# juanaldayparejo/archnemesis-dist

Hardware: AMD Instinct MI355X
Metric: forward-models/sec (10k nu x 100 layers) (higher is better)
Workload: dtype f64; 1 GPU; synthetic correlated-k nadir thermal-emission forward model: 10000 wavenumbers x 100 layers x 8 gases, G=20, k-table 20Px15T (BASELINE configs[1], SURVEY C2); parallelism=replicas x1 (independent forward models)

## Files before the change

### archnemesis_dist_amd/csrc/ansfm_api.hip

```cpp
#include "ansfm_table_kernels.hip.h"
#include "ansfm_rt_params.h"
#include "ansfm_ctx.hip.h"

using namespace ansfm;

extern "C" {

int ansfm_abi_version(void) { return ANSFM_ABI_VERSION; }

int ansfm_create(int device, ansfm_ctx **out)
{
    if (!out) return ANSFM_ERR_INVALID;
    *out = nullptr;
    int ndev = 0;
    if (hipGetDeviceCount(&ndev) != hipSuccess || ndev <= 0 || device < 0 || device >= ndev)
        return ANSFM_ERR_HIP;
    ansfm_ctx *ctx = new ansfm_ctx();
    ctx->device = device;
    if (hipSetDevice(device) != hipSuccess) { delete ctx; return ANSFM_ERR_HIP; }
    if (hipStreamCreateWithFlags(&ctx->own_stream, hipStreamNonBlocking) != hipSuccess) {
        delete ctx;
        return ANSFM_ERR_HIP;
    }
    ctx->stream = ctx->own_stream;
// ... 419 lines not shown
{
    ansfm_ctx *ctx = const_cast<ansfm_ctx *>(cctx);
    CHECK_CTX(ctx);
    if (!applied || !valid_bytes_nonzero) FAIL(ANSFM_ERR_INVALID, "last_merge_order: null argument");
    *applied = ctx->last_merge_ordered ? 1 : 0;
    *valid_bytes_nonzero = 0;
    if (!ctx->last_merge_ordered || ctx->d_flag.bytes < kFlagInts * sizeof(int)) return ANSFM_OK;
    HIPCHK(hipSetDevice(ctx->device));
    unsigned long long v = 0;
    HIPCHK(hipMemcpyAsync(&v, ctx->d_flag.as<int>() + kFlagTileCounter + 8 + 4, sizeof v, hipMemcpyDeviceToHost, ctx->stream));
    HIPCHK(hipStreamSynchronize(ctx->stream));
    *valid_bytes_nonzero = (int64_t)v;
    return ANSFM_OK;
}

int ansfm_last_merge_suffix(const ansfm_ctx *cctx, int64_t *rows, int64_t *rows_of_list_merges)
{
    ansfm_ctx *ctx = const_cast<ansfm_ctx *>(cctx);
    CHECK_CTX(ctx);
    if (!rows || !rows_of_list_merges) FAIL(ANSFM_ERR_INVALID, "last_merge_suffix: null argument");
    *rows = *rows_of_list_merges = 0;
    if (ctx->d_flag.bytes < kFlagInts * sizeof(int)) return ANSFM_OK;
    HIPCHK(hipSetDevice(ctx->device));
    unsigned long long v[kMergeTotals] = {0, 0, 0, 0};
    HIPCHK(hipMemcpyAsync(v, ctx->d_flag.as<int>() + kFlagTileCounter + 8, sizeof v, hipMemcpyDeviceToHost, ctx->stream));
    HIPCHK(hipStreamSynchronize(ctx->stream));
    *rows = (int64_t)v[3];
    *rows_of_list_merges = (int64_t)(v[1] - v[0]) * ctx->last_merge_G;
    return ANSFM_OK;
}

static void launch_w_to_last(hipStream_t st, unsigned n_batch, const double *src, double *dst, int W, int Wpad, int X1, int X2,
                             int swap12, double padval, size_t src_stride = 0, size_t dst_stride = 0)
{
    const int X = X1 * X2;
    dim3 grid((unsigned)(Wpad / 32), (unsigned)((X + 31) / 32), n_batch);
    hipLaunchKernelGGL(k_transpose_w_last, grid, dim3(32, 8), 0, st, src, dst, W, Wpad, X1, X2, swap12, padval, src_stride,
                       dst_stride);
}

static int read_unsorted(ansfm_ctx *ctx, int *flag)
{
    *flag = 0;
    HIPCHK(hipMemcpyAsync(flag, ctx->d_flag.as<int>() + 1, sizeof(int), hipMemcpyDeviceToHost, ctx->stream));
    HIPCHK(hipStreamSynchronize(ctx->stream));
    if (*flag & 2) FAIL(ANSFM_ERR_HIP, "merge kernel: dynamic LDS does not start at address 0 (unexpected code object layout)");
    *flag &= 1;
    return ANSFM_OK;
}

}
// ... 1194 lines not shown
```

### archnemesis_dist_amd/csrc/ansfm_ctx.hip.h

```cpp
#pragma once
#include <hip/hip_runtime.h>
#include <stdio.h>
#include <stdlib.h>
#include <string.h>

#include <algorithm>
#include <cmath>
#include <initializer_list>
#include <memory>
#include <string>
#include <map>
#include <vector>

#pragma GCC visibility push(default)
#include "../../include/ansfm.h"
#pragma GCC visibility pop
#include "ansfm_merge_plan.h"

namespace ansfm {

struct DevBuf {
    void *p = nullptr;
    size_t bytes = 0;
    DevBuf() = default;
// ... 19 lines not shown
    double t_ref = 0, p_ref = 0, s_floor = 0, wn_calc_window = 0, wn_approx_window = 0;
    DevBuf lines;
    std::vector<double> dabs;
    int Nb = 0, nb = 0;
    int first = 0, last = 0, jmax = 0;
    double t_cont = 0, p_cont = 0, wmax = 0;
    DevBuf bins;
};

struct FusedRoute {
    DevBuf ws;
    size_t scratch_bytes = 0;
    int recorded = 0;
    hipEvent_t ev[3] = {nullptr, nullptr, nullptr};
    double ms[2] = {0.0, 0.0};
};

}

using ansfm::DevBuf;
using ansfm::FusedRoute;
using ansfm::LblrtIso;

constexpr int kFlagInts = 32, kFlagTileCounter = 16, kMergeTotals = 4;
static_assert(kFlagTileCounter + 8 + 2 * kMergeTotals <= kFlagInts, "the totals lie inside d_flag");

struct ansfm_ctx {
    int device = 0;
    hipStream_t own_stream = nullptr;
    hipStream_t stream = nullptr;
    std::string err;
    int num_cus = 256;

    int W = 0, Wpad = 0, G = 0, NP = 0, NT = 0, S = 0;
    int monotone = 0;
    int has_boxed = 1;
    std::vector<double> h_wave, h_press, h_temp;
    DevBuf dcont_gas;
    int dcont_gas_L = 0;
    unsigned grad_gas_mask = 0xFFFFFFFFu;
    std::map<const void *, size_t> merge_lds_allowed;
    ansfm::MergePlan last_merge;
    int merge_keys = 64;
    DevBuf merge_hint;
    int merge_hint_parity = 0;
    struct MergeHintKey {
        long source = -1;
// ... 191 lines not shown
```

### archnemesis_dist_amd/csrc/ansfm_merge64.hip.h

```cpp
#pragma once
#include <hip/hip_runtime.h>
#include <stdint.h>
#include "ansfm_merge_common.hip.h"

namespace ansfm {

constexpr unsigned kLdsDG = 0, kLdsGORD = kMaxG * 8, kLdsDGF = (2 * kMaxG + 2) * 8, kLdsA = kLdsDGF + kMaxG * 4;


constexpr unsigned kLdsWT = kLdsA;
static_assert(kLdsA == kMergeLdsTables, "the plan's LDS arithmetic");
typedef double dbl2 __attribute__((ext_vector_type(2)));
constexpr unsigned kRecRow = 64u * 16u, kRecBin = 2u * kRecRow;

struct MergeElem {
    double ai, bc, bn, w;
    int ci, np;
};

struct MergeOrient {
    unsigned rbase, cbase;
    unsigned rsh, csh;
    unsigned inc;
};
// ... 339 lines not shown
#pragma unroll
            for (int j = 0; j < NR; ++j) {
                if (j < merge_rowmajor_sure_cols(NR) || j < G) {
                    MergeElem e;
                    e.ai = a0; e.bc = c[j]; e.w = lds_ld(wa + (unsigned)j * 256u);
                    merge_walk_nodiv(e, ws, rec);
                }
            }
        }
        return;
    }
    double w1[NR], a1;
    merge_rowmajor_weights<NR>(w0, a0, i0, G, mo);
    for (int i = i0; i < G; i += 2) {
        merge_rowmajor_weights<NR>(w1, a1, i + 1 < G ? i + 1 : i, G, mo);
        merge_rowmajor_row<NR>(a0, c, w0, G, ws, rec);
        if (i + 1 < G) {
            merge_rowmajor_weights<NR>(w0, a0, i + 2 < G ? i + 2 : i, G, mo);
            merge_rowmajor_row<NR>(a1, c, w1, G, ws, rec);
        }
    }
}

__device__ __forceinline__ void sort_column(double *X, unsigned char *P, int G, int lane)
{
    for (int g = 0; g < G; ++g) P[g * kWave + lane] = (unsigned char)g;
    for (int i = 1; i < G; ++i) {
        const double key = X[i * kWave + lane];
        const unsigned char pk = P[i * kWave + lane];
        int j = i - 1;
        while (j >= 0 && X[j * kWave + lane] > key) {
            X[(j + 1) * kWave + lane] = X[j * kWave + lane];
            P[(j + 1) * kWave + lane] = P[j * kWave + lane];
            --j;
        }
        X[(j + 1) * kWave + lane] = key;
        P[(j + 1) * kWave + lane] = pk;
    }
}

}
```

### archnemesis_dist_amd/csrc/ansfm_merge_common.hip.h

```cpp
#pragma once
#include <hip/hip_runtime.h>
#include <stdint.h>
#include "ansfm_merge_plan.h"

namespace ansfm {

__device__ __forceinline__ double encode_lnk(double k)
{
    if (k > 0.0) return log(k);
    unsigned long long b = (unsigned long long)__double_as_longlong(k);
    unsigned long long box = 0x7FF8000000000000ULL | (b >> 13);
    return __longlong_as_double((long long)box);
}
__device__ __forceinline__ bool lnk_is_boxed(double x) { return x != x; }
__device__ __forceinline__ double lnk_unbox(double x)
{
    unsigned long long b = (unsigned long long)__double_as_longlong(x);
    return __longlong_as_double((long long)((b & 0x0007FFFFFFFFFFFFULL) << 13));
}

struct LayerInterp {
    int ipl, iph, itl, ith;
    double v, u, dudt;
};
// ... 39 lines not shown
        double klo1 = lnk_unbox(l1), klo2 = lnk_unbox(l2), khi1 = lnk_unbox(h1), khi2 = lnk_unbox(h2);
        kk = (1.0 - v) * (1.0 - u) * klo1 + v * (1.0 - u) * khi1 + v * u * khi2 + (1.0 - v) * u * klo2;
        dk = (-klo1 * (1.0 - v) - khi1 * v + khi2 * v + klo2 * (1.0 - v)) * dudt;
    }
}


struct OverlapParams {
    const double *lnK;
    const double *kin;
    const LayerInterp *li;
    const double *amount;
    const double *del_g;
    double *tau;
    double *scratch;
    int *err_flag;
    unsigned int *tile_counter;
    int W, Wpad, G, NT, S, L, n_models;
    int delg_f32;
    double g_ord[kMaxG + 2];
    const double *lnKg;
    const unsigned char *hint_in;
    unsigned char *hint_out;
};
__host__ __device__ constexpr int gfast_stride(int G) { return (G + 1) & ~1; }
typedef double lnk_pair __attribute__((ext_vector_type(2)));


constexpr int kLoadBatch = 10;

template <bool FROM_K, bool NONNEG = false, bool NOBOX = false>
__device__ __forceinline__ void load_gas(const OverlapParams &p, const LayerInterp &q, int m, int l,
                                         int s, int nu, double *DST, int lane, bool &unsorted)
{
    const int G = p.G;
    const double amt = p.amount[((size_t)m * p.S + s) * p.L + l];
    double prev = NONNEG ? 0.0 : -__builtin_inf();
    if constexpr (FROM_K) {
        const double *src = p.kin + (((size_t)s * p.L + l) * G) * p.Wpad + nu;
        for (int g0 = 0; g0 < G; g0 += kLoadBatch) {
            double r[kLoadBatch];
#pragma unroll
            for (int k = 0; k < kLoadBatch; ++k) {
                const int gi = (g0 + k < G) ? g0 + k : G - 1;
                r[k] = src[(size_t)gi * p.Wpad];
            }
// ... 322 lines not shown
```

### archnemesis_dist_amd/csrc/ansfm_merge_plan.h

```cpp
#pragma once
#include <stddef.h>
#include <stdlib.h>
#include <string.h>

#include <type_traits>

#if defined(__HIPCC__)
#define ANSFM_HD __host__ __device__
#else
#define ANSFM_HD
#endif

namespace ansfm {

constexpr int kWave = 64;
constexpr int kMaxG = 32;

constexpr int kOptTable = 1, kOptBfi = 2, kOptExit = 8, kOptOrient = 16;
constexpr int kMergeOpt = kOptTable | kOptBfi | kOptExit | kOptOrient;
constexpr int kOptLaneRows = 32;
constexpr int kOptRowMajor = 64;
constexpr int kFlagLaneRows = 1, kFlagRowMajor = 2;
constexpr int kFlagTableGfast = 4;
constexpr int kFlagSuffixOff = 8;
ANSFM_HD constexpr bool merge_opt_valid(int opt) { return opt == 0 || (opt & ~kOptTable) == (kOptBfi | kOptExit | kOptOrient); }
ANSFM_HD constexpr int merge_wave_rows(int G, int opt) { return 2 * G + ((opt & kOptOrient) != 0 ? 2 : 1); }
constexpr int kMaxBlockWaves = 8;
ANSFM_HD constexpr unsigned weight_table_bytes(int G) { return (unsigned)(G + 1) * 32u * 8u; }
constexpr int kLaneNV = 2;

constexpr size_t kCuLdsBytes = (size_t)160 * 1024;
constexpr size_t kLdsGranule = 128;
constexpr size_t kMergeLdsTables = (size_t)(2 * kMaxG + 2) * sizeof(double) + kMaxG * sizeof(float);

inline int merge_list_len(int G)
{
    static const int sizes[] = {8, 10, 16, 20, 32};
    for (int v : sizes) if (v >= G) return v;
    return 32;
}
constexpr int kMergeOrderMinList = 16;
constexpr int kSuffixMinList = 16;
template <class F>
auto by_list_len(int G, F &&f)
{
    switch (merge_list_len(G)) {
        case 8: return f(std::integral_constant<int, 8>{});
        case 10: return f(std::integral_constant<int, 10>{});
        case 16: return f(std::integral_constant<int, 16>{});
        case 20: return f(std::integral_constant<int, 20>{});
        default: return f(std::integral_constant<int, 32>{});
    }
}

inline long merge_grid(int num_cus, size_t block_bytes, int max_per_cu, long ntiles)
{
    int per_cu = (int)(kCuLdsBytes / block_bytes);
    if (per_cu < 1) per_cu = 1;
    if (per_cu > max_per_cu) per_cu = max_per_cu;
    long grid = (long)num_cus * per_cu;
    if (grid > ntiles) grid = ntiles;
    return grid < 1 ? 1 : grid;
}

struct MergeSwitches {
    enum Lanes { kLanesUnset, kLanesWavenumbers, kLanesPairs };
    bool walk_records = false;
    bool load_boxtests = false;
    bool legacy = false;
    int keys = 0;
    int waves_per_cu = 0;
    Lanes lanes = kLanesUnset;
    bool rowmajor_off = false;
    bool layout_wave = false;
    bool order_off = false;
    bool suffix_off = false;
};
inline MergeSwitches merge_switches_from_env()
{
    MergeSwitches sw;
    const auto is = [](const char *name, const char *value) { const char *ev = getenv(name); return ev && !strcmp(ev, value); };
    const auto starts = [](const char *name, char c) { const char *ev = getenv(name); return ev && ev[0] == c; };
    sw.walk_records = is("ANSFM_MERGE_WALK", "records");
    sw.load_boxtests = starts("ANSFM_LOAD_BOXTESTS", '1');
    sw.legacy = starts("ANSFM_MERGE_LEGACY", '1');
    if (const char *ev = getenv("ANSFM_MERGE_KEYS")) sw.keys = atoi(ev) == 32 ? 32 : 64;
    if (const char *ev = getenv("ANSFM_WAVES_PER_CU")) sw.waves_per_cu = atoi(ev);
    if (is("ANSFM_MERGE_LANES", "wavenumbers")) sw.lanes = MergeSwitches::kLanesWavenumbers;
    else if (is("ANSFM_MERGE_LANES", "pairs")) sw.lanes = MergeSwitches::kLanesPairs;
    sw.rowmajor_off = starts("ANSFM_MERGE_ROWMAJOR", '0');
    sw.layout_wave = is("ANSFM_TABLE_LAYOUT", "wave");
    sw.order_off = starts("ANSFM_MERGE_ORDER", '0');
    sw.suffix_off = starts("ANSFM_MERGE_SUFFIX", '0');
    return sw;
}

struct MergeCall {
    bool from_k = false;
    bool generic = false;
    bool monotone = false;
    bool has_boxed = true;
    bool delg_f32 = false;
    int merge_keys = 64;
    int G = 0, S = 0, W = 0, Wpad = 0, L = 0, n_models = 0, num_cus = 0;
    double w00 = 0.0, g_ord1 = 0.0;
    bool gfast_copy = false;
    int table_W = 0, table_Wpad = 0, table_G = 0, table_S = 0;
    size_t lds32 = 0;
};

struct MergePlan {
    bool sorted = false, nodiv = false, nobox = false, keys32 = false;
    int opt = 0;
    bool lane_rows = false, rowmajor = false, gfast = false;
    bool suffix = false;
    int lane_nv = 0, flags = 0;
    bool order = false;
    int nwaves = 1;
    size_t lds = 0;
    long grid = 1;
    size_t scratch_bytes_per_block = 0;
    int trims = 0, group_width = 0;
};

inline MergePlan merge_plan(const MergeCall &c, const MergeSwitches &sw)
{
    MergePlan m;
    m.sorted = !c.generic && (c.from_k || c.monotone);
    m.nodiv = m.sorted && c.G >= 2 && c.w00 < c.g_ord1 && !sw.walk_records;
    m.nobox = m.nodiv && !c.from_k && !c.has_boxed && !sw.load_boxtests;
    m.keys32 = m.nodiv && (sw.keys != 0 ? sw.keys : c.merge_keys) == 32;
    const bool trimmed = m.nodiv && !sw.legacy && !m.keys32;
    m.opt = !trimmed ? 0 : c.delg_f32 ? kMergeOpt : (kMergeOpt & ~kOptTable);
    const bool table = (m.opt & kOptTable) != 0;

    const int max_per_cu = sw.waves_per_cu >= 1 && sw.waves_per_cu < kMaxBlockWaves ? sw.waves_per_cu : kMaxBlockWaves;
    const size_t wave_bytes = (size_t)merge_wave_rows(c.G, m.opt) * kWave * sizeof(double);
    const long ntiles = (long)c.n_models * (c.Wpad / kWave) * c.L;
    if (table) {
        const size_t shared_bytes = kMergeLdsTables + weight_table_bytes(c.G);
        const int fit = (int)((kCuLdsBytes - shared_bytes) / wave_bytes);
        m.nwaves = fit < max_per_cu ? fit : max_per_cu;
        m.lds = shared_bytes + (size_t)m.nwaves * wave_bytes;
        const long per_cu = merge_grid(c.num_cus, m.lds, 1, ntiles), needed = (ntiles + m.nwaves - 1) / m.nwaves;
        m.grid = per_cu < needed ? per_cu : needed;
    } else {
        m.nwaves = 1;
        m.lds = m.keys32 ? c.lds32 : wave_bytes + kMergeLdsTables + (m.sorted ? 0 : (size_t)2 * c.G * kWave);
        m.grid = merge_grid(c.num_cus, (m.lds + kLdsGranule - 1) / kLdsGranule * kLdsGranule, max_per_cu, ntiles);
    }
    m.scratch_bytes_per_block = (size_t)m.nwaves * 6 * c.G * kWave * sizeof(double);

    m.lane_rows = m.opt != 0 && (long)c.n_models * c.L < (1L << 24) && sw.lanes != MergeSwitches::kLanesWavenumbers;
    m.lane_nv = m.opt == 0 ? 0 : sw.lanes == MergeSwitches::kLanesPairs ? kLaneNV : 1;
    m.rowmajor = table && !sw.rowmajor_off;
    m.gfast = m.lane_rows && !c.from_k && c.gfast_copy && c.W == c.table_W && c.Wpad == c.table_Wpad && c.G == c.table_G &&
              c.S == c.table_S && !sw.layout_wave;
    m.order = m.rowmajor && m.lane_rows && m.lane_nv == 1 && merge_list_len(c.G) >= kMergeOrderMinList && !sw.order_off;
    m.suffix = m.rowmajor && !sw.suffix_off && merge_list_len(c.G) >= kSuffixMinList;
    m.flags = (m.lane_rows ? kFlagLaneRows : 0) | (m.rowmajor ? kFlagRowMajor : 0) | (m.gfast ? kFlagTableGfast : 0) |
              (m.rowmajor && sw.suffix_off ? kFlagSuffixOff : 0);
    m.trims = m.opt | (m.lane_rows ? kOptLaneRows : 0) | (m.rowmajor ? kOptRowMajor : 0);
    m.group_width = m.lane_rows ? m.lane_nv : 0;
    return m;
}

}
```

### archnemesis_dist_amd/csrc/ansfm_overlap.hip

```cpp
#include "ansfm_overlap_kernels.hip.h"
#include "ansfm_merge32_launch.h"
#include "ansfm_ctx.hip.h"

namespace ansfm {

void merge_params(ansfm_ctx *ctx, OverlapParams &p, const double *kin, int W, int Wpad, int G, int S, int L, int n_models,
                  const LayerInterp *li, const double *amount, const double *del_g_dev, const double *del_g_host, double *tau)
{
    p.lnK = ctx->lnK.as<double>();
    p.kin = kin;
    p.li = li;
    p.amount = amount;
    p.del_g = del_g_dev;
    p.tau = tau;
    p.err_flag = ctx->d_flag.as<int>() + 1;
    p.tile_counter = reinterpret_cast<unsigned int *>(ctx->d_flag.as<int>() + kFlagTileCounter);
    p.W = W; p.Wpad = Wpad; p.G = G; p.NT = ctx->NT; p.S = S; p.L = L; p.n_models = n_models;
    p.delg_f32 = ctx->delg_f32;
    double acc = 0.0;
    float accf = 0.0f;
    p.g_ord[0] = 0.0;
    for (int g = 0; g < G; ++g) {
        if (ctx->delg_f32) { accf += (float)del_g_host[g]; p.g_ord[g + 1] = (double)accf; }
        else { acc += del_g_host[g]; p.g_ord[g + 1] = acc; }
    }
    p.g_ord[G] = 1.0;
    p.g_ord[G + 1] = __builtin_nan("");
}

int merge_launch_begin(ansfm_ctx *ctx, const OverlapParams &p, long grid, std::initializer_list<MergeWorkspace> workspaces)
{
    for (const MergeWorkspace &w : workspaces) HIPCHK(w.buf->reserve((size_t)grid * w.bytes_per_block));
    HIPCHK(hipMemsetAsync(p.tile_counter, 0, (8 + 2 * kMergeTotals) * sizeof(unsigned int), ctx->stream));
    return ANSFM_OK;
}

using MergeKernel = void (*)(OverlapParams, int, int);

template <int D, bool FK, bool W32>
static MergeKernel overlap_kernel_of(const MergePlan &m)
{
    constexpr int kTrimmed = W32 ? kMergeOpt : (kMergeOpt & ~kOptTable);
    if (m.opt == kTrimmed) return m.nobox ? k_ck_overlap<D, false, W32, true, true, true, kTrimmed> : k_ck_overlap<D, FK, W32, true, true, false, kTrimmed>;
    if (m.opt != 0) return nullptr;
    if (m.nodiv) return m.nobox ? k_ck_overlap<D, false, W32, true, true, true> : k_ck_overlap<D, FK, W32, true, true>;
    return m.sorted ? k_ck_overlap<D, FK, W32, true> : k_ck_overlap<D, FK, W32, false>;
}

template <bool FK>
static MergeKernel overlap_kernel_fk(const MergePlan &m, bool w32, int G)
// ... 6 lines not shown

static MergeKernel overlap_kernel(const MergePlan &m, bool from_k, bool w32, int G)
{
    return from_k ? overlap_kernel_fk<true>(m, w32, G) : overlap_kernel_fk<false>(m, w32, G);
}

int launch_overlap(ansfm_ctx *ctx, bool from_k, const double *kin, int W, int Wpad, int G, int S,
                   int L, int n_models, const LayerInterp *li, const double *amount,
                   const double *del_g_dev, const double *del_g_host, double *tau, bool generic)
{
    OverlapParams p;
    memset(&p, 0, sizeof p);
    merge_params(ctx, p, kin, W, Wpad, G, S, L, n_models, li, amount, del_g_dev, del_g_host, tau);
    const bool w32 = ctx->delg_f32 != 0;
    MergeCall c;
    c.from_k = from_k; c.generic = generic; c.monotone = ctx->monotone != 0; c.has_boxed = ctx->has_boxed != 0; c.delg_f32 = w32;
    c.merge_keys = ctx->merge_keys;
    c.G = G; c.S = S; c.W = W; c.Wpad = Wpad; c.L = L; c.n_models = n_models; c.num_cus = ctx->num_cus;
    c.w00 = w32 ? (double)((float)del_g_host[0] * (float)del_g_host[0]) : del_g_host[0] * del_g_host[0];
    c.g_ord1 = p.g_ord[1];
    c.gfast_copy = ctx->lnKg_bytes != 0 && !ctx->is_lbl;
    c.table_W = ctx->W; c.table_Wpad = ctx->Wpad; c.table_G = ctx->G; c.table_S = ctx->S;
    c.lds32 = overlap32_lds_bytes(G, w32);
    const MergePlan m = merge_plan(c, merge_switches_from_env());

    const int rc = merge_launch_begin(ctx, p, m.grid, {{&ctx->scratch, m.scratch_bytes_per_block}});
    if (rc) return rc;
    p.scratch = ctx->scratch.as<double>();
    if (m.gfast) p.lnKg = ctx->lnKg.as<double>();
    ctx->last_merge = m;
    ctx->last_merge_G = G;
    ctx->last_merge_ordered = false;
    ansfm_ctx::MergeHintKey key;
    bool valid = false;
    if (m.order) {
        key.source = from_k ? 0 : ctx->table_generation;
        key.W = W; key.Wpad = Wpad; key.R = n_models * L; key.S = S; key.G = G;
        HIPCHK(ctx->merge_hint.reserve((size_t)2 * Wpad));
        valid = key == ctx->merge_hint_key;
        if (!valid) HIPCHK(hipMemsetAsync(ctx->merge_hint.p, 0, (size_t)2 * Wpad, ctx->stream));
        p.hint_in = ctx->merge_hint.as<unsigned char>() + (size_t)ctx->merge_hint_parity * Wpad;
        p.hint_out = ctx->merge_hint.as<unsigned char>() + (size_t)(1 - ctx->merge_hint_parity) * Wpad;
    }
    if (m.keys32) {
        HIPCHK(launch_overlap32(p, from_k, (unsigned)m.grid, ctx->stream));
        return ANSFM_OK;
// ... 22 lines not shown
```

### archnemesis_dist_amd/csrc/ansfm_overlap_kernels.hip.h

```cpp
#pragma once
#include "ansfm_merge64.hip.h"

namespace ansfm {


template <bool FROM_K, bool NOBOX, int OPT>
__device__ __forceinline__ void load_cell(const OverlapParams &p, int lane_rows, bool gfast, const LaneRow &lr, const LayerInterp &q, int m,
                                          int l, int s, int nu, double *DST, int lane, bool &unsorted)
{
    if constexpr (OPT != 0) {
        if (lane_rows != 0) {
            if (!FROM_K && gfast) load_gas_rows<FROM_K, NOBOX, true>(p, lr, s, DST, lane, unsorted);
            else load_gas_rows<FROM_K, NOBOX, false>(p, lr, s, DST, lane, unsorted);
            return;
        }
    }
    load_gas<FROM_K, false, NOBOX>(p, q, m, l, s, nu, DST, lane, unsorted);
}

template <int NR, bool FROM_K, bool W32, bool SORTED = true, bool NODIV = false, bool NOBOX = false, int OPT = 0>
__global__ __launch_bounds__((OPT & kOptTable) != 0 ? kWave * kMaxBlockWaves : kWave) __attribute__((amdgpu_waves_per_eu(1, 2)))
void k_ck_overlap(OverlapParams p, int flags, int lane_nv)
{
    static_assert(OPT == 0 || (SORTED && NODIV), "the fast path");
    static_assert(merge_opt_valid(OPT), "OPT == 0 || (OPT & ~kOptTable) == (kOptBfi | kOptExit | kOptOrient)");
    constexpr bool kTable = (OPT & kOptTable) != 0, kOrient = (OPT & kOptOrient) != 0;
    static_assert(!kTable || W32, "the weight table holds float32 products only (launch_overlap)");
    constexpr bool kSuffix = kTable && NR >= kSuffixMinList;
    const int lane_rows = kTable ? (flags & kFlagLaneRows) : flags;
    const bool gfast = !FROM_K && OPT != 0 && (flags & kFlagTableGfast) != 0;
    const unsigned nvs = lane_nv == 1 ? 0u : kLaneNVShift;
    unsigned n_rowmajor = 0, n_merged = 0;
    unsigned n_suffix = 0;
    const bool ordered = kTable && p.hint_in != nullptr;
    unsigned n_hints = 0;
    extern __shared__ double smem[];
    const int lane = kTable ? (int)(threadIdx.x & 63u) : (int)threadIdx.x;
    const int wv = kTable ? __builtin_amdgcn_readfirstlane((int)(threadIdx.x >> 6)) : 0;
    const int nwv = kTable ? (int)(blockDim.x >> 6) : 1;
    const int G = p.G;
    double *DG = smem;
    double *GORD = DG + kMaxG;
    double *A = reinterpret_cast<double *>(reinterpret_cast<char *>(GORD + kMaxG + 2) + kMaxG * sizeof(float));
    if constexpr (kTable) {
        double *WT = A;
        for (int idx = (int)threadIdx.x; idx < (G + 1) * 32; idx += (int)blockDim.x) {
            const int row = idx & 31, col = idx >> 5;
            double w = 0.0;
            if (row < G && col < G) w = (double)((float)p.del_g[row] * (float)p.del_g[col]);
            WT[idx] = w;
        }
        A = WT + (G + 1) * 32 + (size_t)wv * merge_wave_rows(G, OPT) * kWave;
    }
    double *B = A + (kOrient ? G + 1 : G) * kWave;
    unsigned char *PA = reinterpret_cast<unsigned char *>(B + (G + 1) * kWave);
    unsigned char *PB = PA + G * kWave;
    if (wv == 0 && lane < G) {
        DG[lane] = p.del_g[lane];
        const_cast<float *>(delg_f32_table(DG))[lane] = (float)p.del_g[lane];
    }
    if (wv == 0 && lane < G + 2) GORD[lane] = p.g_ord[lane];
    const double HUGE_KEY = __longlong_as_double(0x7FE0000000000000LL);
    B[G * kWave + lane] = HUGE_KEY;
    if constexpr (kOrient) A[G * kWave + lane] = HUGE_KEY;
    __syncthreads();
    double wsum = 0.0;
    for (int g = 0; g < G; ++g) wsum += DG[g];
    const double wtot = wsum * wsum;

    double *rec = p.scratch + ((size_t)blockIdx.x * nwv + wv) * 6 * G * kWave;
    TileQueue tq;
    tq.init();
    for (;;) {
        int vt = 0, m = 0, l = 0;
        LaneRow lr{};
// ... 16 lines not shown
            if (!tq.next(p, lane, vt, m, l)) break;
        }
        const int nu = vt * kWave + lane;
        LayerInterp q;
        if constexpr (!FROM_K) q = p.li[(size_t)m * p.L + l];
        bool unsorted = false;
        unsigned pattern = 0;

        load_cell<FROM_K, NOBOX, OPT>(p, lane_rows, gfast, lr, q, m, l, 0, nu, A, lane, unsorted);
        double alast = A[(G - 1) * kWave + lane];
        if constexpr (!SORTED) sort_column(A, PA, G, lane);
        for (int s = 1; s < p.S; ++s) {
            load_cell<FROM_K, NOBOX, OPT>(p, lane_rows, gfast, lr, q, m, l, s, nu, B, lane, unsorted);
            if constexpr (SORTED)
                if (__builtin_amdgcn_ballot_w64(unsorted) != 0) break;
            const double blast = B[(G - 1) * kWave + lane];
            if constexpr (!SORTED) sort_column(B, PB, G, lane);
            if constexpr (SORTED) alast = A[(G - 1) * kWave + lane];
            bool takeB, keepA;
            if (s == 1) { takeB = (alast <= 0.0); keepA = !takeB && (blast <= 0.0); }
            else { keepA = (blast <= 0.0); takeB = !keepA && (alast <= 0.0); }
            const bool do_merge = !(takeB | keepA);
            bool walked = false;
            int walked_rows = 0;
            if (takeB) {
                for (int g = 0; g < G; ++g) A[g * kWave + lane] = B[g * kWave + lane];
                if constexpr (!SORTED) {
                    for (int g = 0; g < G; ++g) PA[g * kWave + lane] = PB[g * kWave + lane];
                    alast = blast;
                }
            }
            if (do_merge) {
                double R[NR];
                MergeOrient mo{};
                if constexpr (kOrient) {
                    bool swapped = blast > alast;
                    if (__builtin_amdgcn_ballot_w64(swapped) != 0) {
                        double prev = A[lane];
                        for (int g = 1; g < G; ++g) {
                            const double v = A[g * kWave + lane];
                            swapped &= (v >= prev);
                            prev = v;
                        }
                    }
                    mo = merge_orient(lds_addr(A + lane), lds_addr(B + lane), swapped);
                    merge_init<NR>(R, G, mo, HUGE_KEY);
// ... 13 lines not shown
                    walked = i0 == 0;
                    if (i0 != 0) walked_rows = G - i0;
                    pattern |= lane_passes && s <= 8 ? 0x100u >> s : 0u;
                }
                if (!kTable || i0 != 0) {
                merge_fetch<W32, SORTED, OPT>(R[0], lane, A, B, DG, e0, PA, PB, mo);
                ws = walk_begin(GORD, lane);
                const bool partial = kSuffix && i0 < G;
                const int nloop = partial ? G * i0 : G * G - (G - 1);
                constexpr int kPer = 2;
                for (int n = nloop / kPer; n > 0; --n) {
                    merge_step<NR, W32, false, SORTED, NODIV, NR, OPT>(R, e0, e1, ws, lane, A, B, DG, GORD, rec, PA, PB, mo);
                    merge_step<NR, W32, false, SORTED, NODIV, NR, OPT>(R, e1, e0, ws, lane, A, B, DG, GORD, rec, PA, PB, mo);
                }
                if (!partial || (nloop & 1) != 0)
                merge_step<NR, W32, false, SORTED, NODIV, NR, OPT>(R, e0, e1, ws, lane, A, B, DG, GORD, rec, PA, PB, mo);
                if (!partial) {
                if (((G ^ NR) & 1) != 0) { const MergeElem t = e0; e0 = e1; e1 = t; }
                merge_peel<NR - 1, NR, W32, SORTED, NODIV, OPT>(R, e0, e1, ws, G, lane, A, B, DG, GORD, rec, PA, PB, mo);
                }
                }
                if constexpr (kTable) {
                    if (i0 < G) {
                        if (i0 == 0) ws = walk_begin(GORD, lane);
                        merge_rowmajor<NR>(i0, G, mo, ws, rec);
                    }
                }
                if constexpr (NODIV) {
                    const int ig = walk_bins(ws, GORD);
                    for (int g0 = 0; g0 < G; g0 += kLoadBatch) {
                        double r[kLoadBatch];
#pragma unroll
                        for (int k = 0; k < kLoadBatch; ++k)
                            r[k] = gld<double>(rec, (unsigned)((g0 + k < G) ? g0 + k : G - 1) * (kWave * 8u) + (unsigned)lane * 8u);
#pragma unroll
                        for (int k = 0; k < kLoadBatch; ++k) {
                            const int b = g0 + k;
                            if (b < G) {
                                double outv = 0.0;
                                if (b < ig) outv = fast_div(r[k], GORD[b + 1] - GORD[b]);
                                else if (b == ig) outv = (b == G - 1) ? fast_div(ws.kacc, ws.gd - GORD[G - 1]) : ws.kacc;
                                A[b * kWave + lane] = outv;
                            }
                        }
                    }
                } else {
                double ck = 0.0, cs = 0.0;
                const int ig = walk_bins(ws, GORD);
                constexpr int kRB = 5;
                for (int b0 = 0; b0 < G; b0 += kRB) {
                    double rka[kRB], rs1[kRB], rgd[kRB];
                    unsigned rcd[kRB];
#pragma unroll
                    for (int k = 0; k < kRB; ++k) {
                        const int bi = (b0 + k < G) ? b0 + k : G - 1;
                        const unsigned ro = (unsigned)bi * kRecBin + (unsigned)lane * 16u;
                        const dbl2 v0 = gld<dbl2>(rec, ro), v1 = gld<dbl2>(rec, ro + kRecRow);
                        rka[k] = v0.x; rs1[k] = v0.y; rgd[k] = v1.x; rcd[k] = (unsigned)__double_as_longlong(v1.y);
                    }
#pragma unroll
                    for (int k = 0; k < kRB; ++k) {
                        const int b = b0 + k;
                        if (b < G) {
// ... 12 lines not shown
                                const double kb = (ck + ka) + frac * cw;
                                const double sb = (cs + s1) + frac * w;
                                outv = fast_div(kb, sb);
                                ck = (1.0 - frac) * cw;
                                cs = (1.0 - frac) * w;
                            } else if (b == ig) {
                                const double kb = ck + ws.kacc, sb = cs + ws.sum1;
                                outv = (b == G - 1) ? fast_div(kb, sb) : kb;
                            }
                            gst<double>(rec, (unsigned)b * kRecBin + (unsigned)lane * 16u, outv);
                        }
                    }
                }
                for (int g0 = 0; g0 < G; g0 += kLoadBatch) {
                    double r[kLoadBatch];
#pragma unroll
                    for (int k = 0; k < kLoadBatch; ++k)
                        r[k] = gld<double>(rec, (unsigned)((g0 + k < G) ? g0 + k : G - 1) * kRecBin + (unsigned)lane * 16u);
#pragma unroll
                    for (int k = 0; k < kLoadBatch; ++k)
                        if (g0 + k < G) A[(g0 + k) * kWave + lane] = r[k];
                }
                }
                if constexpr (!SORTED) {
                    for (int g = 0; g < G; ++g) PA[g * kWave + lane] = (unsigned char)g;
                    alast = A[(G - 1) * kWave + lane];
                }
            }
            if constexpr (kTable) {
                n_merged += __builtin_amdgcn_ballot_w64(do_merge) != 0 ? 1u : 0u;
                n_rowmajor += __builtin_amdgcn_ballot_w64(walked) != 0 ? 1u : 0u;
                const unsigned long long some = __builtin_amdgcn_ballot_w64(walked_rows != 0);
                if (some != 0) n_suffix += (unsigned)__builtin_amdgcn_readlane(walked_rows, __builtin_ctzll(some));
            }
        }
        if constexpr (OPT != 0) {
            if (lane_rows != 0) {
                if (unsorted) atomicOr(p.err_flag, 1);
                double *outr = p.tau + ((size_t)lr.row * G) * p.Wpad + lr.nu;
                for (int g = 0; g < G; ++g) outr[(size_t)g * p.Wpad] = A[g * kWave + lane];
                if constexpr (kTable) {
                    if (ordered && lr.row == (((unsigned)p.n_models * (unsigned)p.L) >> 1) && lr.nu < p.W)
                        p.hint_out[lr.nu] = (unsigned char)pattern;
                }
                continue;
            }
        }
        double *out = p.tau + (((size_t)m * p.L + l) * G) * p.Wpad + nu;
        if constexpr (SORTED) {
            if (unsorted) atomicOr(p.err_flag, 1);
            for (int g = 0; g < G; ++g) out[(size_t)g * p.Wpad] = A[g * kWave + lane];
        } else {
            for (int g = 0; g < G; ++g) out[(size_t)PA[g * kWave + lane] * p.Wpad] = A[g * kWave + lane];
        }
    }
    if constexpr (kTable) {
        unsigned long long *cnt = reinterpret_cast<unsigned long long *>(p.tile_counter + 8);
        if (lane == 0) {
            atomicAdd(cnt, (unsigned long long)n_rowmajor);
            atomicAdd(cnt + 1, (unsigned long long)n_merged);
            if (ordered) atomicAdd(cnt + 2, (unsigned long long)n_hints);
            if (n_suffix != 0) atomicAdd(cnt + 3, (unsigned long long)n_suffix);
        }
    }
}

}
```

### archnemesis_dist_amd/engine.py

```python
import contextlib
import ctypes as C
import os
import numpy as np

from . import _lib

_f8 = np.float64


def _np(a, dtype=_f8):
    return None if a is None else np.ascontiguousarray(a, dtype=dtype)


def _is_f32(a):
    return getattr(a, "dtype", None) == np.float32


def _ptr(a):
    if a is None:
        return None
    if isinstance(a, np.ndarray):
        return a.ctypes.data_as(C.c_void_p)
    return C.c_void_p(a.data_ptr())

# ... 219 lines not shown
        w = C.c_int()
        self._check(self._lib.ansfm_last_merge_group_width(self._ctx, C.byref(w)), "last_merge_group_width")
        return int(w.value)

    def ktable_gfast(self):
        p, b = C.c_int(), C.c_int64()
        self._check(self._lib.ansfm_ktable_gfast(self._ctx, C.byref(p), C.byref(b)), "ktable_gfast")
        return bool(p.value), int(b.value)

    def last_merge_table_layout(self):
        g = C.c_int()
        self._check(self._lib.ansfm_last_merge_table_layout(self._ctx, C.byref(g)), "last_merge_table_layout")
        return bool(g.value)

    def last_merge_rowmajor(self):
        m, t = C.c_int64(), C.c_int64()
        self._check(self._lib.ansfm_last_merge_rowmajor(self._ctx, C.byref(m), C.byref(t)), "last_merge_rowmajor")
        return int(m.value), int(t.value)

    def last_merge_suffix(self):
        r, t = C.c_int64(), C.c_int64()
        self._check(self._lib.ansfm_last_merge_suffix(self._ctx, C.byref(r), C.byref(t)), "last_merge_suffix")
        return int(r.value), int(t.value)

    def last_merge_order(self):
        a, n = C.c_int(), C.c_int64()
        self._check(self._lib.ansfm_last_merge_order(self._ctx, C.byref(a), C.byref(n)), "last_merge_order")
        return bool(a.value), int(n.value)

    def calc_k(self, press, temp, grad=False):
        press = _np(press); temp = _np(temp)
        W, G, NP, NT, S = self.dims
        L = press.shape[0]
        k = np.empty((W, G, L, S)); dk = np.empty((W, G, L, S)) if grad else None
        self._check(self._lib.ansfm_calc_k(self._ctx, L, _ptr(press), _ptr(temp), _ptr(k), _ptr(dk)), "calc_k")
        return (k, dk) if grad else k

    def k_overlap(self, del_g, k_w_g_l_gas, amount_layer):
        self.set_f32_semantics(getattr(self, "grid_f32", False), _is_f32(del_g))
        del_g = _np(del_g); k = _np(k_w_g_l_gas); am = _np(amount_layer)
        W, G, L, S = k.shape
        if am.shape != (S, L):
            raise ValueError("amount_layer must be (NGAS, NLAYER)")
        tau = np.empty((W, G, L))
        self._check(self._lib.ansfm_k_overlap(self._ctx, W, G, L, S, _ptr(del_g), _ptr(k), _ptr(am), _ptr(tau)),
                    "k_overlap")
# ... 1345 lines not shown
```

### include/ansfm.h

```cpp
#ifndef ANSFM_H
#define ANSFM_H

#include <stdint.h>

#ifdef __cplusplus
extern "C" {
#endif

#define ANSFM_ABI_VERSION 1

#define ANSFM_OK 0
#define ANSFM_ERR_INVALID 1
#define ANSFM_ERR_HIP 2
#define ANSFM_ERR_NOTABLE 3
#define ANSFM_ERR_UNSORTED 4
#define ANSFM_ERR_UNSUPPORTED 5

#define ANSFM_MAX_NG 32
#define ANSFM_MAX_CONT_GRAD_SLOTS 48

typedef struct ansfm_ctx ansfm_ctx;

int ansfm_abi_version(void);

int ansfm_create(int device, ansfm_ctx **ctx);
void ansfm_destroy(ansfm_ctx *ctx);
const char *ansfm_last_error(const ansfm_ctx *ctx);

int ansfm_set_stream(ansfm_ctx *ctx, void *hip_stream);
int ansfm_synchronize(ansfm_ctx *ctx);

int ansfm_set_f32_semantics(ansfm_ctx *ctx, int grid_f32, int delg_f32);

int ansfm_upload_ktable(ansfm_ctx *ctx, int W, int G, int NP, int NT, int S, const double *K,
                        const double *PRESS, const double *TEMP, const double *WAVE,
                        const double *DELG);
int ansfm_upload_ktable_dev(ansfm_ctx *ctx, int W, int G, int NP, int NT, int S,
                            const double *K_dev, const double *PRESS, const double *TEMP,
                            const double *WAVE, const double *DELG);
int ansfm_ktable_info(const ansfm_ctx *ctx, int64_t dims[5], int *monotone);
int ansfm_ktable_has_boxed(const ansfm_ctx *ctx, int *has_boxed);
int ansfm_last_merge_launch(const ansfm_ctx *ctx, int *waves_per_block, int *trims);
int ansfm_last_merge_rowmajor(const ansfm_ctx *ctx, int64_t *merges, int64_t *merges_total);
int ansfm_last_merge_suffix(const ansfm_ctx *ctx, int64_t *rows, int64_t *rows_of_list_merges);
int ansfm_last_merge_group_width(const ansfm_ctx *ctx, int *width);
int ansfm_ktable_gfast(const ansfm_ctx *ctx, int *present, int64_t *bytes);
int ansfm_last_merge_table_layout(const ansfm_ctx *ctx, int *gfast);
int ansfm_last_merge_order(const ansfm_ctx *ctx, int *applied, int64_t *valid_bytes_nonzero);

int ansfm_upload_lbltable(ansfm_ctx *ctx, int W, int NP, int NT, int S, const double *K,
                          const double *PRESS, const double *TEMP, int temp2d, const double *WAVE);
int ansfm_calc_klbl(ansfm_ctx *ctx, int L, const double *press, const double *temp, double *k_out,
                    double *dkdT_out);

int ansfm_ktable_file_header(const char *path, int64_t dims[4], int32_t ids[2], double hdr[3], double *wave,
                             float *g_ord, float *del_g, float *press, float *temp);
int ansfm_upload_ktable_files(ansfm_ctx *ctx, int S, const char *const *paths, double wavemin, double wavemax);
int ansfm_ktable_grids(const ansfm_ctx *ctx, double *WAVE, double *PRESS, double *TEMP, double *DELG);
int ansfm_lbltable_file_header(const char *path, int64_t dims[3], int32_t ids[2], double hdr[2], double *wave,
                               float *press, float *temp);
int ansfm_upload_lbltable_files(ansfm_ctx *ctx, int S, const char *const *paths, double wavemin, double wavemax);

int ansfm_kdist_bins(ansfm_ctx *ctx, int ncalc, const double *wavecalc, const double *kabs, int nbin,
                     const double *vbinmin, const double *vbinmax, const double *wcen, int nfilmax,
                     const int32_t *nfil, const double *dfil, const double *afil, int NG, const double *g_ord,
                     double *kout);

// ... 366 lines not shown
```

Before: 301.3 forward-models/s.

## Precompute static bin-crossing tables for random-overlap merge walk

On the host, it precomputes which (i,j) product cells cross each g-ordinate bin boundary, plus the split coefficients, for the float32 weight table. This is valid because the weights depend only on del_g. The kernel stores these tables and reciprocal bin widths in LDS and walks the merge with a uniform per-row bitmask, instead of doing data-dependent comparisons against the cumulative g-ordinates. Division by bin width is replaced with a refined reciprocal multiply. The change adds extra LDS per block, which may reduce waves per CU, and it only applies when G is at least 16 and the table is valid.

```diff
diff --git a/archnemesis_dist_amd/csrc/ansfm_api.hip b/archnemesis_dist_amd/csrc/ansfm_api.hip
--- a/archnemesis_dist_amd/csrc/ansfm_api.hip
+++ b/archnemesis_dist_amd/csrc/ansfm_api.hip
@@ -465,11 +465,27 @@
     *rows = *rows_of_list_merges = 0;
     if (ctx->d_flag.bytes < kFlagInts * sizeof(int)) return ANSFM_OK;
     HIPCHK(hipSetDevice(ctx->device));
-    unsigned long long v[kMergeTotals] = {0, 0, 0, 0};
+    unsigned long long v[4] = {0, 0, 0, 0};
     HIPCHK(hipMemcpyAsync(v, ctx->d_flag.as<int>() + kFlagTileCounter + 8, sizeof v, hipMemcpyDeviceToHost, ctx->stream));
     HIPCHK(hipStreamSynchronize(ctx->stream));
     *rows = (int64_t)v[3];
     *rows_of_list_merges = (int64_t)(v[1] - v[0]) * ctx->last_merge_G;
+    return ANSFM_OK;
+}
+
+int ansfm_last_merge_static(const ansfm_ctx *cctx, int64_t *merges, int *valid)
+{
+    ansfm_ctx *ctx = const_cast<ansfm_ctx *>(cctx);
+    CHECK_CTX(ctx);
+    if (!merges || !valid) FAIL(ANSFM_ERR_INVALID, "last_merge_static: null argument");
+    *merges = 0;
+    *valid = ctx->last_merge.static_tables ? 1 : 0;
+    if (ctx->d_flag.bytes < kFlagInts * sizeof(int)) return ANSFM_OK;
+    HIPCHK(hipSetDevice(ctx->device));
+    unsigned long long v = 0;
+    HIPCHK(hipMemcpyAsync(&v, ctx->d_flag.as<int>() + kFlagTileCounter + 8 + 8, sizeof v, hipMemcpyDeviceToHost, ctx->stream));
+    HIPCHK(hipStreamSynchronize(ctx->stream));
+    *merges = (int64_t)v;
     return ANSFM_OK;
 }
 
diff --git a/archnemesis_dist_amd/csrc/ansfm_ctx.hip.h b/archnemesis_dist_amd/csrc/ansfm_ctx.hip.h
--- a/archnemesis_dist_amd/csrc/ansfm_ctx.hip.h
+++ b/archnemesis_dist_amd/csrc/ansfm_ctx.hip.h
@@ -65,7 +65,7 @@
 using ansfm::FusedRoute;
 using ansfm::LblrtIso;
 
-constexpr int kFlagInts = 32, kFlagTileCounter = 16, kMergeTotals = 4;
+constexpr int kFlagInts = 40, kFlagTileCounter = 16, kMergeTotals = 5;
 static_assert(kFlagTileCounter + 8 + 2 * kMergeTotals <= kFlagInts, "the totals lie inside d_flag");
 
 struct ansfm_ctx {
diff --git a/archnemesis_dist_amd/csrc/ansfm_merge64.hip.h b/archnemesis_dist_amd/csrc/ansfm_merge64.hip.h
--- a/archnemesis_dist_amd/csrc/ansfm_merge64.hip.h
+++ b/archnemesis_dist_amd/csrc/ansfm_merge64.hip.h
@@ -385,6 +385,111 @@
     }
 }
 
+constexpr unsigned kStaticRD = 0, kStaticC = kMaxG * 16u, kStaticMask = 2u * kMaxG * 16u;
+static_assert(kStaticMask + kMaxG * 4u == kMergeStaticLds, "the plan's LDS arithmetic");
+__device__ __forceinline__ unsigned merge_static_base(int G) { return kLdsWT + weight_table_bytes(G); }
+typedef __attribute__((address_space(3))) dbl2 lds_dbl2;
+typedef __attribute__((address_space(3))) unsigned lds_uint;
+__device__ __forceinline__ dbl2 lds_ld2(unsigned a) { return *(const lds_dbl2 *)(size_t)a; }
+__device__ __forceinline__ double recip_div(double n, dbl2 rd)
+{
+    const double q = n * rd.x;
+    return fma(fma(-rd.y, q, n), rd.x, q);
+}
+__device__ __forceinline__ void merge_static_fill(const OverlapParams &p, int G, int lane)
+{
+    const unsigned sb = merge_static_base(G);
+    if (lane < G) {
+        const double d = p.g_ord[lane + 1] - p.g_ord[lane];
+        double r = __builtin_amdgcn_rcp(d);
+        r = fma(fma(-d, r, 1.0), r, r);
+        r = fma(fma(-d, r, 1.0), r, r);
+        *(lds_dbl2 *)(size_t)(sb + kStaticRD + (unsigned)lane * 16u) = dbl2{r, d};
+    }
+    if (lane < kMaxG) {
+        *(lds_dbl2 *)(size_t)(sb + kStaticC + (unsigned)lane * 16u) = dbl2{p.st.c1[lane], p.st.c2[lane]};
+        *(lds_uint *)(size_t)(sb + kStaticMask + (unsigned)lane * 4u) = p.st.rowmask[lane];
+    }
+}
+struct StaticWalk {
+    double kacc;
+    dbl2 cc;
+    unsigned caddr;
+    unsigned oaddr;
+};
+template <bool TEST>
+__device__ __forceinline__ void merge_static_elem(int j, double cv, double w, unsigned mask, StaticWalk &sw)
+{
+    if (TEST && ((mask >> j) & 1u) != 0) {
+        lds_st(sw.oaddr, fma(sw.cc.x, cv, sw.kacc));
+        sw.kacc = sw.cc.y * cv;
+        sw.oaddr += 512u;
+        sw.caddr += 16u;
+        sw.cc = lds_ld2(sw.caddr);
+    } else
+        sw.kacc = fma(cv, w, sw.kacc);
+}
+template <int NR>
+__device__ __forceinline__ void merge_static_row(double ai, const double (&c)[NR], const double (&w)[NR], unsigned wa, unsigned mask,
+                                                 int G, StaticWalk &sw)
+{
+    constexpr int kSure = merge_rowmajor_sure_cols(NR);
+    constexpr unsigned kInner = ((1u << kSure) - 1u) & ~1u;
+    const auto weight = [&](int j) { if constexpr (NR > 20) return lds_ld(wa + (unsigned)j * 256u); else return w[j]; };
+    merge_static_elem<true>(0, ai + c[0], weight(0), mask, sw);
+    if ((mask & kInner) == 0) {
+#pragma unroll
+        for (int j = 1; j < kSure; ++j) merge_static_elem<false>(j, ai + c[j], weight(j), mask, sw);
+    } else {
+#pragma unroll
+        for (int j = 1; j < kSure; ++j) merge_static_elem<true>(j, ai + c[j], weight(j), mask, sw);
+    }
+#pragma unroll
+    for (int j = kSure; j < NR; ++j)
+        if (j < G) merge_static_elem<true>(j, ai + c[j], weight(j), mask, sw);
+}
+__device__ __forceinline__ unsigned merge_static_mask(unsigned sb, int i)
+{
+    return *(const lds_uint *)(size_t)(sb + kStaticMask + ((unsigned)i << 2));
+}
+template <int NR>
+__device__ __forceinline__ double merge_rowmajor_static(int G, const MergeOrient &mo, unsigned a_lane)
+{
+    const unsigned sb = merge_static_base(G);
+    double c[NR], w0[NR], a0;
+#pragma unroll
+    for (int j = 0; j < NR; ++j) c[j] = lds_ld(mo.cbase + (unsigned)(j < G ? j : 0) * 512u);
+    StaticWalk sw;
+    sw.kacc = 0.0;
+    sw.caddr = sb + kStaticC;
+    sw.cc = lds_ld2(sw.caddr);
+    sw.oaddr = a_lane;
+    if constexpr (NR > 20) {
+        for (int i = 0; i < G; ++i) {
+            a0 = lds_ld(mo.rbase + ((unsigned)i << 9));
+            const unsigned m = (unsigned)__builtin_amdgcn_readfirstlane((int)merge_static_mask(sb, i));
+            merge_static_row<NR>(a0, c, c, kLdsWT + ((unsigned)i << 3), m, G, sw);
+        }
+        return sw.kacc;
+    }
+    double w1[NR], a1;
+    unsigned m0 = merge_static_mask(sb, 0), m1;
+    merge_rowmajor_weights<NR>(w0, a0, 0, G, mo);
+    for (int i = 0; i < G; i += 2) {
+        const int i1 = i + 1 < G ? i + 1 : i;
+        m1 = merge_static_mask(sb, i1);
+        merge_rowmajor_weights<NR>(w1, a1, i1, G, mo);
+        merge_static_row<NR>(a0, c, w0, 0u, (unsigned)__builtin_amdgcn_readfirstlane((int)m0), G, sw);
+        if (i + 1 < G) {
+            const int i2 = i + 2 < G ? i + 2 : i;
+            m0 = merge_static_mask(sb, i2);
+            merge_rowmajor_weights<NR>(w0, a0, i2, G, mo);
+            merge_static_row<NR>(a1, c, w1, 0u, (unsigned)__builtin_amdgcn_readfirstlane((int)m1), G, sw);
+        }
+    }
+    return sw.kacc;
+}
+
 __device__ __forceinline__ void sort_column(double *X, unsigned char *P, int G, int lane)
 {
     for (int g = 0; g < G; ++g) P[g * kWave + lane] = (unsigned char)g;
diff --git a/archnemesis_dist_amd/csrc/ansfm_merge_common.hip.h b/archnemesis_dist_amd/csrc/ansfm_merge_common.hip.h
--- a/archnemesis_dist_amd/csrc/ansfm_merge_common.hip.h
+++ b/archnemesis_dist_amd/csrc/ansfm_merge_common.hip.h
@@ -85,6 +85,7 @@
     const double *lnKg;
     const unsigned char *hint_in;
     unsigned char *hint_out;
+    MergeStatic st;
 };
 __host__ __device__ constexpr int gfast_stride(int G) { return (G + 1) & ~1; }
 typedef double lnk_pair __attribute__((ext_vector_type(2)));
diff --git a/archnemesis_dist_amd/csrc/ansfm_merge_plan.h b/archnemesis_dist_amd/csrc/ansfm_merge_plan.h
--- a/archnemesis_dist_amd/csrc/ansfm_merge_plan.h
+++ b/archnemesis_dist_amd/csrc/ansfm_merge_plan.h
@@ -1,4 +1,5 @@
 #pragma once
+#include <float.h>
 #include <stddef.h>
 #include <stdlib.h>
 #include <string.h>
@@ -23,6 +24,7 @@
 constexpr int kFlagLaneRows = 1, kFlagRowMajor = 2;
 constexpr int kFlagTableGfast = 4;
 constexpr int kFlagSuffixOff = 8;
+constexpr int kFlagStatic = 16, kFlagStaticOff = 32;
 ANSFM_HD constexpr bool merge_opt_valid(int opt) { return opt == 0 || (opt & ~kOptTable) == (kOptBfi | kOptExit | kOptOrient); }
 ANSFM_HD constexpr int merge_wave_rows(int G, int opt) { return 2 * G + ((opt & kOptOrient) != 0 ? 2 : 1); }
 constexpr int kMaxBlockWaves = 8;
@@ -41,6 +43,59 @@
 }
 constexpr int kMergeOrderMinList = 16;
 constexpr int kSuffixMinList = 16;
+constexpr int kStaticMinList = 16;
+constexpr size_t kMergeStaticLds = (size_t)kMaxG * 16 + (size_t)kMaxG * 16 + (size_t)kMaxG * 4;
+
+inline void merge_g_ord(const double *del_g, int G, bool delg_f32, double *g_ord)
+{
+    double acc = 0.0;
+    float accf = 0.0f;
+    g_ord[0] = 0.0;
+    for (int g = 0; g < G; ++g) {
+        if (delg_f32) { accf += (float)del_g[g]; g_ord[g + 1] = (double)accf; }
+        else { acc += del_g[g]; g_ord[g + 1] = acc; }
+    }
+    g_ord[G] = 1.0;
+    g_ord[G + 1] = __builtin_nan("");
+}
+
+struct MergeStatic {
+    unsigned rowmask[kMaxG];
+    double c1[kMaxG], c2[kMaxG];
+    double gd_end, last_width;
+    int nbins;
+    int valid;
+};
+inline void merge_static_build(const double *del_g, const double *g_ord, int G, MergeStatic &s)
+{
+    memset(&s, 0, sizeof s);
+    if (G < 2 || G > kMaxG) return;
+    const auto plain = [](float v) { const float m = v < 0.0f ? -v : v; return v == 0.0f || (m >= FLT_MIN && m <= FLT_MAX); };
+    bool ok = true;
+    double gd = 0.0;
+    int ig = 0;
+    for (int i = 0; i < G; ++i) {
+        for (int j = 0; j < G; ++j) {
+            const float fi = (float)del_g[i], fj = (float)del_g[j];
+            const float wf = fi * fj;
+            ok = ok && plain(fi) && plain(fj) && plain(wf);
+            const double w = (double)wf;
+            const double gdn = gd + w;
+            if (ig < G && gdn >= g_ord[ig + 1]) {
+                ok = ok && ig <= i;
+                s.rowmask[i] |= 1u << j;
+                s.c1[ig] = g_ord[ig + 1] - gd;
+                s.c2[ig] = gdn - g_ord[ig + 1];
+                ++ig;
+            }
+            gd = gdn;
+        }
+    }
+    s.nbins = ig;
+    s.gd_end = gd;
+    s.last_width = gd - g_ord[G - 1];
+    s.valid = ok ? 1 : 0;
+}
 template <class F>
 auto by_list_len(int G, F &&f)
 {
@@ -75,6 +130,7 @@
     bool layout_wave = false;
     bool order_off = false;
     bool suffix_off = false;
+    bool static_off = false;
 };
 inline MergeSwitches merge_switches_from_env()
 {
@@ -92,6 +148,7 @@
     sw.layout_wave = is("ANSFM_TABLE_LAYOUT", "wave");
     sw.order_off = starts("ANSFM_MERGE_ORDER", '0');
     sw.suffix_off = starts("ANSFM_MERGE_SUFFIX", '0');
+    sw.static_off = starts("ANSFM_MERGE_STATIC", '0');
     return sw;
 }
 
@@ -107,6 +164,7 @@
     bool gfast_copy = false;
     int table_W = 0, table_Wpad = 0, table_G = 0, table_S = 0;
     size_t lds32 = 0;
+    bool static_valid = false;
 };
 
 struct MergePlan {
@@ -114,6 +172,7 @@
     int opt = 0;
     bool lane_rows = false, rowmajor = false, gfast = false;
     bool suffix = false;
+    bool static_tables = false, static_walk = false;
     int lane_nv = 0, flags = 0;
     bool order = false;
     int nwaves = 1;
@@ -138,7 +197,8 @@
     const size_t wave_bytes = (size_t)merge_wave_rows(c.G, m.opt) * kWave * sizeof(double);
     const long ntiles = (long)c.n_models * (c.Wpad / kWave) * c.L;
     if (table) {
-        const size_t shared_bytes = kMergeLdsTables + weight_table_bytes(c.G);
+        m.static_tables = c.static_valid && merge_list_len(c.G) >= kStaticMinList;
+        const size_t shared_bytes = kMergeLdsTables + weight_table_bytes(c.G) + (m.static_tables ? kMergeStaticLds : 0);
         const int fit = (int)((kCuLdsBytes - shared_bytes) / wave_bytes);
         m.nwaves = fit < max_per_cu ? fit : max_per_cu;
         m.lds = shared_bytes + (size_t)m.nwaves * wave_bytes;
@@ -158,8 +218,10 @@
               c.S == c.table_S && !sw.layout_wave;
     m.order = m.rowmajor && m.lane_rows && m.lane_nv == 1 && merge_list_len(c.G) >= kMergeOrderMinList && !sw.order_off;
     m.suffix = m.rowmajor && !sw.suffix_off && merge_list_len(c.G) >= kSuffixMinList;
+    m.static_walk = m.static_tables && m.rowmajor && !sw.static_off;
     m.flags = (m.lane_rows ? kFlagLaneRows : 0) | (m.rowmajor ? kFlagRowMajor : 0) | (m.gfast ? kFlagTableGfast : 0) |
-              (m.rowmajor && sw.suffix_off ? kFlagSuffixOff : 0);
+              (m.rowmajor && sw.suffix_off ? kFlagSuffixOff : 0) | (m.static_tables ? kFlagStatic : 0) |
+              (m.static_tables && !m.static_walk ? kFlagStaticOff : 0);
     m.trims = m.opt | (m.lane_rows ? kOptLaneRows : 0) | (m.rowmajor ? kOptRowMajor : 0);
     m.group_width = m.lane_rows ? m.lane_nv : 0;
     return m;
diff --git a/archnemesis_dist_amd/csrc/ansfm_overlap.hip b/archnemesis_dist_amd/csrc/ansfm_overlap.hip
--- a/archnemesis_dist_amd/csrc/ansfm_overlap.hip
+++ b/archnemesis_dist_amd/csrc/ansfm_overlap.hip
@@ -17,15 +17,7 @@
     p.tile_counter = reinterpret_cast<unsigned int *>(ctx->d_flag.as<int>() + kFlagTileCounter);
     p.W = W; p.Wpad = Wpad; p.G = G; p.NT = ctx->NT; p.S = S; p.L = L; p.n_models = n_models;
     p.delg_f32 = ctx->delg_f32;
-    double acc = 0.0;
-    float accf = 0.0f;
-    p.g_ord[0] = 0.0;
-    for (int g = 0; g < G; ++g) {
-        if (ctx->delg_f32) { accf += (float)del_g_host[g]; p.g_ord[g + 1] = (double)accf; }
-        else { acc += del_g_host[g]; p.g_ord[g + 1] = acc; }
-    }
-    p.g_ord[G] = 1.0;
-    p.g_ord[G + 1] = __builtin_nan("");
+    merge_g_ord(del_g_host, G, ctx->delg_f32 != 0, p.g_ord);
 }
 
 int merge_launch_begin(ansfm_ctx *ctx, const OverlapParams &p, long grid, std::initializer_list<MergeWorkspace> workspaces)
@@ -78,6 +70,8 @@
     c.gfast_copy = ctx->lnKg_bytes != 0 && !ctx->is_lbl;
     c.table_W = ctx->W; c.table_Wpad = ctx->Wpad; c.table_G = ctx->G; c.table_S = ctx->S;
     c.lds32 = overlap32_lds_bytes(G, w32);
+    if (w32) merge_static_build(del_g_host, p.g_ord, G, p.st);
+    c.static_valid = p.st.valid != 0;
     const MergePlan m = merge_plan(c, merge_switches_from_env());
 
     const int rc = merge_launch_begin(ctx, p, m.grid, {{&ctx->scratch, m.scratch_bytes_per_block}});
diff --git a/archnemesis_dist_amd/csrc/ansfm_overlap_kernels.hip.h b/archnemesis_dist_amd/csrc/ansfm_overlap_kernels.hip.h
--- a/archnemesis_dist_amd/csrc/ansfm_overlap_kernels.hip.h
+++ b/archnemesis_dist_amd/csrc/ansfm_overlap_kernels.hip.h
@@ -27,11 +27,15 @@
     constexpr bool kTable = (OPT & kOptTable) != 0, kOrient = (OPT & kOptOrient) != 0;
     static_assert(!kTable || W32, "the weight table holds float32 products only (launch_overlap)");
     constexpr bool kSuffix = kTable && NR >= kSuffixMinList;
+    constexpr bool kStatic = kTable && NR >= kStaticMinList;
+    const bool st_tables = kStatic && (flags & kFlagStatic) != 0;
+    const bool st_walk = kStatic && (flags & (kFlagStatic | kFlagStaticOff)) == kFlagStatic;
     const int lane_rows = kTable ? (flags & kFlagLaneRows) : flags;
     const bool gfast = !FROM_K && OPT != 0 && (flags & kFlagTableGfast) != 0;
     const unsigned nvs = lane_nv == 1 ? 0u : kLaneNVShift;
     unsigned n_rowmajor = 0, n_merged = 0;
     unsigned n_suffix = 0;
+    unsigned n_static = 0;
     const bool ordered = kTable && p.hint_in != nullptr;
     unsigned n_hints = 0;
     extern __shared__ double smem[];
@@ -51,6 +55,12 @@
             WT[idx] = w;
         }
         A = WT + (G + 1) * 32 + (size_t)wv * merge_wave_rows(G, OPT) * kWave;
+        if constexpr (kStatic) {
+            if (st_tables) {
+                A += kMergeStaticLds / sizeof(double);
+                if (wv == 0) merge_static_fill(p, G, lane);
+            }
+        }
     }
     double *B = A + (kOrient ? G + 1 : G) * kWave;
     unsigned char *PA = reinterpret_cast<unsigned char *>(B + (G + 1) * kWave);
@@ -113,6 +123,7 @@
             else { keepA = (blast <= 0.0); takeB = !keepA && (alast <= 0.0); }
             const bool do_merge = !(takeB | keepA);
             bool walked = false;
+            bool walked_static = false;
             int walked_rows = 0;
             if (takeB) {
                 for (int g = 0; g < G; ++g) A[g * kWave + lane] = B[g * kWave + lane];
@@ -172,10 +183,41 @@
                 }
                 if constexpr (kTable) {
                     if (i0 < G) {
-                        if (i0 == 0) ws = walk_begin(GORD, lane);
-                        merge_rowmajor<NR>(i0, G, mo, ws, rec);
-                    }
-                }
+                        if constexpr (kStatic) walked_static = i0 == 0 && st_walk;
+                        if (!walked_static) {
+                            if (i0 == 0) ws = walk_begin(GORD, lane);
+                            merge_rowmajor<NR>(i0, G, mo, ws, rec);
+                        }
+                    }
+                }
+                if constexpr (kStatic) {
+                if (walked_static) {
+                    const unsigned a_lane = lds_addr(A + lane), sb = merge_static_base(G);
+                    const double kacc = merge_rowmajor_static<NR>(G, mo, a_lane);
+                    const int ig = p.st.nbins;
+                    for (int g0 = 0; g0 < G; g0 += kLoadBatch) {
+                        double r[kLoadBatch];
+                        dbl2 rd[kLoadBatch];
+#pragma unroll
+                        for (int k = 0; k < kLoadBatch; ++k) {
+                            const unsigned b = (unsigned)((g0 + k < G) ? g0 + k : G - 1);
+                            r[k] = lds_ld(a_lane + b * 512u);
+                            rd[k] = lds_ld2(sb + kStaticRD + b * 16u);
+                        }
+#pragma unroll
+                        for (int k = 0; k < kLoadBatch; ++k) {
+                            const int b = g0 + k;
+                            if (b < G) {
+                                double outv = 0.0;
+                                if (b < ig) outv = recip_div(r[k], rd[k]);
+                                else if (b == ig) outv = (b == G - 1) ? fast_div(kacc, p.st.last_width) : kacc;
+                                A[b * kWave + lane] = outv;
+                            }
+                        }
+                    }
+                }
+                }
+                if (!walked_static) {
                 if constexpr (NODIV) {
                     const int ig = walk_bins(ws, GORD);
                     for (int g0 = 0; g0 < G; g0 += kLoadBatch) {
@@ -188,7 +230,10 @@
                             const int b = g0 + k;
                             if (b < G) {
                                 double outv = 0.0;
-                                if (b < ig) outv = fast_div(r[k], GORD[b + 1] - GORD[b]);
+                                if (b < ig) {
+                                    if (st_tables) outv = recip_div(r[k], lds_ld2(merge_static_base(G) + kStaticRD + (unsigned)b * 16u));
+                                    else outv = fast_div(r[k], GORD[b + 1] - GORD[b]);
+                                }
                                 else if (b == ig) outv = (b == G - 1) ? fast_div(ws.kacc, ws.gd - GORD[G - 1]) : ws.kacc;
                                 A[b * kWave + lane] = outv;
                             }
@@ -247,6 +292,7 @@
                         if (g0 + k < G) A[(g0 + k) * kWave + lane] = r[k];
                 }
                 }
+                }
                 if constexpr (!SORTED) {
                     for (int g = 0; g < G; ++g) PA[g * kWave + lane] = (unsigned char)g;
                     alast = A[(G - 1) * kWave + lane];
@@ -255,6 +301,7 @@
             if constexpr (kTable) {
                 n_merged += __builtin_amdgcn_ballot_w64(do_merge) != 0 ? 1u : 0u;
                 n_rowmajor += __builtin_amdgcn_ballot_w64(walked) != 0 ? 1u : 0u;
+                if constexpr (kStatic) n_static += __builtin_amdgcn_ballot_w64(walked_static) != 0 ? 1u : 0u;
                 const unsigned long long some = __builtin_amdgcn_ballot_w64(walked_rows != 0);
                 if (some != 0) n_suffix += (unsigned)__builtin_amdgcn_readlane(walked_rows, __builtin_ctzll(some));
             }
@@ -286,6 +333,7 @@
             atomicAdd(cnt + 1, (unsigned long long)n_merged);
             if (ordered) atomicAdd(cnt + 2, (unsigned long long)n_hints);
             if (n_suffix != 0) atomicAdd(cnt + 3, (unsigned long long)n_suffix);
+            if (n_static != 0) atomicAdd(cnt + 4, (unsigned long long)n_static);
         }
     }
 }
diff --git a/archnemesis_dist_amd/engine.py b/archnemesis_dist_amd/engine.py
--- a/archnemesis_dist_amd/engine.py
+++ b/archnemesis_dist_amd/engine.py
@@ -265,6 +265,11 @@
         r, t = C.c_int64(), C.c_int64()
         self._check(self._lib.ansfm_last_merge_suffix(self._ctx, C.byref(r), C.byref(t)), "last_merge_suffix")
         return int(r.value), int(t.value)
+
+    def last_merge_static(self):
+        m, v = C.c_int64(), C.c_int()
+        self._check(self._lib.ansfm_last_merge_static(self._ctx, C.byref(m), C.byref(v)), "last_merge_static")
+        return int(m.value), bool(v.value)
 
     def last_merge_order(self):
         a, n = C.c_int(), C.c_int64()
diff --git a/include/ansfm.h b/include/ansfm.h
--- a/include/ansfm.h
+++ b/include/ansfm.h
@@ -43,6 +43,7 @@
 int ansfm_last_merge_launch(const ansfm_ctx *ctx, int *waves_per_block, int *trims);
 int ansfm_last_merge_rowmajor(const ansfm_ctx *ctx, int64_t *merges, int64_t *merges_total);
 int ansfm_last_merge_suffix(const ansfm_ctx *ctx, int64_t *rows, int64_t *rows_of_list_merges);
+int ansfm_last_merge_static(const ansfm_ctx *ctx, int64_t *merges, int *valid);
 int ansfm_last_merge_group_width(const ansfm_ctx *ctx, int *width);
 int ansfm_ktable_gfast(const ansfm_ctx *ctx, int *present, int64_t *bytes);
 int ansfm_last_merge_table_layout(const ansfm_ctx *ctx, int *gfast);
```

New measurement: 312.4 forward-models/s (median of 6 runs). 3.7% higher.
